# tuanggolt/hyperdrive

Hardware: AMD Instinct MI355X
Metric: verified consensus msgs/sec (secp256k1) at 1/2/4/8 MI355X; % INT32 VALU peak (higher is better)
Workload: dtype u32 (256-bit modular integer arithmetic)

## Files before the change

hyperdrive_amd/_lib.py:

```python
from __future__ import annotations

import atexit
import ctypes
import os
import weakref

HERE = os.path.dirname(os.path.abspath(__file__))
LIB_PATH = os.environ.get("HD_LIB", os.path.join(HERE, "_lib", "libhdverify.so"))

HD_OK = 0
HD_EINVAL = -1
HD_ENOMEM = -2
HD_EDEVICE = -3
HD_ECAP = -4
HD_EAGAIN = -5

c_u8p = ctypes.POINTER(ctypes.c_uint8)
c_i8p = ctypes.POINTER(ctypes.c_int8)
c_i64p = ctypes.POINTER(ctypes.c_int64)
c_u32p = ctypes.POINTER(ctypes.c_uint32)
c_i32p = ctypes.POINTER(ctypes.c_int32)


class HdBatch(ctypes.Structure):
# ... 87 lines not shown
                ("done", ctypes.c_void_p)]


SIGNATURES = {
    "hd_ctx_create": (ctypes.c_int, [ctypes.c_int, ctypes.POINTER(ctypes.c_void_p)]),
    "hd_ctx_destroy": (ctypes.c_int, [ctypes.c_void_p]),
    "hd_ctx_set_pubkey_format": (ctypes.c_int, [ctypes.c_void_p, ctypes.c_int]),
    "hd_set_signatories": (ctypes.c_int, [ctypes.c_void_p, ctypes.c_void_p, ctypes.c_uint32]),
    "hd_ctx_set_fastpath": (ctypes.c_int, [ctypes.c_void_p, ctypes.c_int]),
    "hd_ctx_fastpath_stats": (ctypes.c_int, [ctypes.c_void_p, ctypes.POINTER(ctypes.c_uint32),
                                             ctypes.POINTER(ctypes.c_uint32)]),
    "hd_ctx_foreign_stats": (ctypes.c_int, [ctypes.c_void_p, ctypes.POINTER(ctypes.c_uint32),
                                            ctypes.POINTER(ctypes.c_uint32), ctypes.POINTER(ctypes.c_uint32)]),
    "hd_ctx_dedup_stats": (ctypes.c_int, [ctypes.c_void_p, ctypes.POINTER(ctypes.c_uint64),
                                          ctypes.POINTER(ctypes.c_uint64)]),
    "hd_ctx_fastpath_geometry": (ctypes.c_int, [ctypes.c_void_p, ctypes.POINTER(ctypes.c_int),
                                                ctypes.POINTER(ctypes.c_int), ctypes.POINTER(ctypes.c_int)]),
    "hd_ctx_profile": (ctypes.c_int, [ctypes.c_void_p, ctypes.c_int]),
    "hd_ctx_set_variant": (ctypes.c_int, [ctypes.c_void_p, ctypes.c_int, ctypes.c_int]),
    "hd_ctx_get_variant": (ctypes.c_int, [ctypes.c_void_p, ctypes.c_int, ctypes.POINTER(ctypes.c_int)]),
    "hd_ctx_profile_read": (ctypes.c_int, [ctypes.c_void_p, ctypes.POINTER(ctypes.c_uint32),
                                           ctypes.POINTER(ctypes.c_double), ctypes.POINTER(ctypes.c_uint32),
                                           ctypes.POINTER(ctypes.c_double)]),
    "hd_verify_batch": (ctypes.c_int, [ctypes.c_void_p, ctypes.POINTER(HdBatch), ctypes.c_void_p,
                                       ctypes.c_void_p, ctypes.c_void_p]),
    "hd_verify_batch_device": (ctypes.c_int, [ctypes.c_void_p, ctypes.POINTER(HdBatch), ctypes.c_void_p,
                                              ctypes.c_void_p, ctypes.c_void_p, ctypes.c_void_p, ctypes.c_void_p]),
    "hd_authenticate_batch_device": (ctypes.c_int, [ctypes.c_void_p, ctypes.POINTER(HdBatch), ctypes.c_void_p,
                                                    ctypes.c_void_p]),
    "hd_verify_submit": (ctypes.c_int, [ctypes.c_void_p, ctypes.POINTER(HdBatch), ctypes.c_void_p, ctypes.c_void_p,
# ... 174 lines not shown
```

hyperdrive_amd/csrc/hd_dedup.h:

```cpp
#pragma once
#include "hd_common.h"

namespace hd {

#define HD_DD_PROBES 8u
#define HD_DD_EMPTY 0xFFFFFFFFu
#define HD_DD_REPEAT 0x80000000u
#define HD_DD_FINAL 0xC0000000u
#define HD_DD_INDEX 0x3FFFFFFFu
#define HD_DD_MAX_N (1u << 30)

struct DdKey {
    int64_t height, round;
    uint32_t value[8], from[8], r[8], s[8];
    uint32_t v;
};

HD bool dd_key_equal(const DdKey& a, const DdKey& b) {
    uint32_t d = (uint32_t)(a.height != b.height) | (uint32_t)(a.round != b.round) | (a.v ^ b.v);
    HD_UNROLL for (int k = 0; k < 8; k++)
        d |= (a.value[k] ^ b.value[k]) | (a.from[k] ^ b.from[k]) | (a.r[k] ^ b.r[k]) | (a.s[k] ^ b.s[k]);
    return d == 0;
}

HD void dd_key_load(DdKey& k, const int64_t* height, const int64_t* round, const uint8_t* value32,
                    const uint8_t* digest32, const uint8_t* from32, const uint8_t* sig65, size_t i, size_t n) {
    if (digest32) {
        k.height = k.round = 0;
        load_row32_be(k.value, digest32, i);
    } else {
        k.height = height[i];
        k.round = round[i];
        load_row32_be(k.value, value32, i);
    }
    load_row32_be(k.from, from32, i);
    load_sig65(k.r, k.s, k.v, sig65, i, n);
}

HD uint32_t dd_hash(const DdKey& k) {
    uint32_t h = k.r[0] * 0x9E3779B1u;
    h = (h ^ k.r[7]) * 0x85EBCA6Bu;
    h = (h ^ (h >> 15) ^ k.s[0]) * 0xC2B2AE35u;
    h = (h ^ k.s[7]) * 0x27D4EB2Fu;
    h = (h ^ (h >> 13) ^ k.from[0]) * 0x165667B1u;
    h = (h ^ k.from[7]) * 0x9E3779B1u;
    return h ^ (h >> 16);
}

HD uint32_t dd_table_words(uint32_t n) {
    uint32_t w = 1024u;
    while (w < 4u * (uint64_t)n && w < 0x80000000u) w <<= 1;
    return w;
}

}
```

hyperdrive_amd/csrc/hd_fastverify.hip:

```cpp
#include <hip/hip_runtime.h>

#include <algorithm>
#include <cstdio>
#include <cstdlib>
#include <cstring>
#include <string>
#include <map>
#include <mutex>
#include <unordered_map>
#include <vector>

#include "../../include/hd_verify.h"
#include "hd_fixedbase.h"
#include "hd_dedup.h"
#include "hd_scmont.h"
#include "hd_internal.h"
#include "hd_verify_msg.h"

using namespace hd;

struct FbWork {
    const gp* gtab = nullptr;
    uint32_t nslots = 0;
    uint32_t max_slots = 0;
// ... 1 lines not shown
    std::vector<gp*> chunks;
    ge* base = nullptr;
    ge* pub = nullptr;
    uint32_t* state = nullptr;
    int32_t* adm_slot = nullptr;
    bool map_ok = true;
    size_t cap_adm_slot = 0;
    uint32_t* list = nullptr;
    uint32_t* counts = nullptr;
    uint32_t* zr = nullptr;
    struct Scratch {
        uint32_t* rows = nullptr;
        size_t cap_rows = 0;
        uint32_t* dtab = nullptr;
        size_t cap_dtab = 0;
        uint32_t* slow = nullptr;
        size_t cap_slow = 0;
        uint32_t* count = nullptr;
        uint32_t* slow2 = nullptr;
        size_t cap_slow2 = 0;
        hipEvent_t done = nullptr;
        hipStream_t stream = nullptr;
        bool used = false;
    };
    static constexpr int NSCRATCH = 3;
    Scratch sc[NSCRATCH];
    int next = 0;
    int last_set = -1;
    uint32_t* nr_host = nullptr;
    uint32_t* nr_dev = nullptr;
    uint32_t* est_host = nullptr;
    uint32_t* est_dev = nullptr;
    unsigned long long* dstats = nullptr;
    hipEvent_t done = nullptr;
    hipStream_t last = nullptr;
    bool any = false;
    bool steady = false;
    bool prof = false;
    std::vector<hipEvent_t> ev_call, ev_sums;
    size_t n_call = 0, n_sums = 0;
    std::unordered_map<std::string, uint32_t> slot_of;
    std::vector<uint32_t> free_slots;
    uint32_t used = 1;
    int wp = HD_FB_W;
    int last_k = 8;
    double budget = 0;
    size_t bytes = 0;
    uint32_t* fdict = nullptr;
// ... 74 lines not shown
    if (p == 1) __builtin_amdgcn_s_setprio(1);
    else if (p == 2) __builtin_amdgcn_s_setprio(2);
    else if (p >= 3) __builtin_amdgcn_s_setprio(3);
}

#define HD_REF_NEG 0x80000000u
#define HD_REF_ZERO 0x40000000u
#define HD_REF_IDX 0x3FFFFFFFu
template <int W>
HD uint32_t fb_ref(int d, int w) {
    const uint32_t ad = (uint32_t)(d < 0 ? -d : d);
    const uint32_t base = (uint32_t)w * FbL<W>::N;
    return d == 0 ? (base | HD_REF_ZERO) : ((base + ad - 1) | (d < 0 ? HD_REF_NEG : 0u));
}

__global__ __launch_bounds__(256) void k_fast_prep(DevBatch b, const uint8_t* __restrict__ digest_in,
                                                   const uint32_t* __restrict__ state,
                                                   const int32_t* __restrict__ adm_slot, AdmIndex ix,
                                                   uint32_t n_adm, SplitRows rows, const uint32_t* __restrict__ fdict,
                                                   uint32_t* __restrict__ fhit, uint32_t fbase,
                                                   uint32_t* __restrict__ dtab, uint32_t dmask) {
    wave_prio(rows.prio);
    const uint32_t i = blockIdx.x * blockDim.x + threadIdx.x;
    const uint32_t n = b.n;
    const bool present = i < n;
    FastSrc src{b, present ? i : 0u, digest_in};
    const uint32_t type = present ? src.type() : 0u;
    uint32_t code = HD_NEEDS_SLOW, slot = 0, rep = HD_DD_EMPTY;
    int32_t idx = -1;
    sc r, s, m;
    if (!present) {
    } else if (type < 1 || type > 3) {
        code = V_BAD_TYPE;
    } else {
        uint32_t from_be[8];
        src.from_words(from_be);
        idx = n_adm ? adm_index_find(ix, from_be) : -1;
        int32_t sl = idx >= 0 ? adm_slot[idx] : -1;
        if (idx < 0 && fdict) {
            sl = fdict_find(fdict, from_be);
            if (sl >= 0) idx = -2;
        }
        if (sl >= 0 && state[sl] == HD_FB_READY) {
            slot = (uint32_t)sl;
            if (idx == -2) atomicAdd(&fhit[sl - (int32_t)fbase], 1u);
            FastIn in;
            DdKey me;
            me.height = me.round = 0;
            if (digest_in) {
                load_row32_be(in.digest_be, digest_in, i);
                HD_UNROLL for (int k = 0; k < 8; k++) me.value[k] = in.digest_be[k];
            } else {
                src.value_words(me.value);
                me.height = b.height[i];
                me.round = b.round[i];
                if (type == T_PROPOSE)
                    sha256_propose(in.digest_be, me.height, me.round, b.valid_round ? b.valid_round[i] : -1, me.value);
                else
                    sha256_vote(in.digest_be, me.height, me.round, me.value);
            }
            src.sig(in.r_be, in.s_be, in.v);
            in.ready = true;
            fe x;
            uint8_t o;
            if (fast_prefix(o, r, s, m, x, in)) {
                code = HD_FAST_LIVE;
                if (dtab && type != T_PROPOSE) {
                    HD_UNROLL for (int k = 0; k < 8; k++) {
                        me.from[k] = from_be[k];
                        me.r[k] = in.r_be[k];
                        me.s[k] = in.s_be[k];
                    }
                    me.v = in.v;
                    const uint32_t h = dd_hash(me);
                    HD_NOUNROLL for (uint32_t p = 0; p < HD_DD_PROBES; p++) {
                        const uint32_t cur = atomicCAS(&dtab[(h + p) & dmask], HD_DD_EMPTY, i);
                        if (cur == HD_DD_EMPTY) break;
                        DdKey other;
                        dd_key_load(other, b.height, b.round, b.value32, digest_in, b.from32, b.sig65, cur, n);
                        if (dd_key_equal(me, other)) {
                            rep = cur;
                            break;
                        }
                    }
                }
            } else {
                code = o;
            }
        }
    }
    const bool live = code == HD_FAST_LIVE;
    const bool distinct = live && rep == HD_DD_EMPTY;
    __shared__ uint32_t s_cnt[4], s_base;
    const uint32_t lane = threadIdx.x & 63u, wv = threadIdx.x >> 6;
    const unsigned long long bd = __ballot(distinct), br = __ballot(live && !distinct);
// ... 798 lines not shown
    if (const char* m = getenv("HD_FB_MAX_BYTES")) f->budget = atof(m);
    f->max_slots = (uint32_t)std::max(1.0, std::min(1e6, f->budget / fb_slot_bytes(f->wp)));
    FBCHK(hipMalloc(&f->counts, 8), "fb counts");
    FBCHK(hipMalloc(&f->zr, fb_run_scratch_bytes(ctx)), "fb builder scratch");
    FBCHK(hipHostMalloc((void**)&f->nr_host, 4, hipHostMallocMapped | hipHostMallocCoherent), "fb ready count");
    *f->nr_host = 0xFFFFFFFFu;
    FBCHK(hipHostGetDevicePointer((void**)&f->nr_dev, f->nr_host, 0), "fb ready count map");
    FBCHK(hipHostMalloc((void**)&f->est_host, 16, hipHostMallocMapped | hipHostMallocCoherent), "fb list estimate");
    f->est_host[0] = f->est_host[1] = f->est_host[2] = f->est_host[3] = 0xFFFFFFFFu;
    FBCHK(hipHostGetDevicePointer((void**)&f->est_dev, f->est_host, 0), "fb list estimate map");
    FBCHK(hipHostMalloc((void**)&f->fpend_host, 8, hipHostMallocMapped | hipHostMallocCoherent), "fb foreign claims");
    f->fpend_host[0] = f->fpend_host[1] = 0;
    FBCHK(hipHostGetDevicePointer((void**)&f->fpend_dev, f->fpend_host, 0), "fb foreign claims map");
    FBCHK(hipMalloc(&f->dstats, 16), "fb repeat counters");
    FBCHK(hipMemset(f->dstats, 0, 16), "fb repeat counters clear");
    int rc = fb_alloc_slots(ctx);
    if (rc) return rc;
    return fb_g_table(ctx, &f->gtab);
}

const gp* hd_fb_gtab(const hd_ctx* ctx) { return ctx && ctx->fb ? ctx->fb->gtab : nullptr; }

void hd_fb_release(hd_ctx* ctx) {
    if (!ctx || !ctx->fb) return;
    FbWork* f = ctx->fb;
    fb_free_tables(ctx);
    if (f->done) (void)hipEventDestroy(f->done);
    for (hipEvent_t e : f->ev_call) (void)hipEventDestroy(e);
    for (hipEvent_t e : f->ev_sums) (void)hipEventDestroy(e);
    for (auto& sc : f->sc) {
        if (sc.done) (void)hipEventDestroy(sc.done);
        void* sp[] = {sc.rows, sc.slow, sc.count, sc.slow2, sc.dtab};
        for (void* p : sp)
            if (p) (void)hipFree(p);
    }
    void* ptrs[] = {f->counts, f->adm_slot, f->zr, f->fdict, f->fnext, f->fhit, f->fkey, f->dstats};
    for (void* p : ptrs)
        if (p) (void)hipFree(p);
    if (f->nr_host) (void)hipHostFree(f->nr_host);
    if (f->est_host) (void)hipHostFree(f->est_host);
    if (f->fpend_host) (void)hipHostFree(f->fpend_host);
    delete f;
    ctx->fb = nullptr;
}

static int split_k_for(const hd_ctx* ctx, uint32_t n) {
    const int k = ctx->var[HD_VAR_SPLIT_K];
    if (k > 0) return k;
    uint64_t lanes = n;
    if (const volatile uint32_t* est = ctx->fb->est_host) {
        const uint32_t seen = est[2], of = est[3];
// ... 190 lines not shown
    const int pf = ctx->var[HD_VAR_SUM_PREFETCH];
    if (w == 0) w = (uint64_t)n < 2ull * 3 * 4 * 64 * (uint64_t)std::max(ctx->n_cu, 1) ? 4 : 3;
    if (pf == 2) {
        if (w == 2) k_fast_sums<2, WP, 2><<<blocks, 256, 0, s>>>(n, gtab, tab, rows);
        else k_fast_sums<3, WP, 2><<<blocks, 256, 0, s>>>(n, gtab, tab, rows);
    } else {
        if (w == 2) k_fast_sums<2, WP, 1><<<blocks, 256, 0, s>>>(n, gtab, tab, rows);
        else if (w == 4) k_fast_sums<4, WP, 0><<<blocks, 256, 0, s>>>(n, gtab, tab, rows);
        else k_fast_sums<3, WP, 1><<<blocks, 256, 0, s>>>(n, gtab, tab, rows);
    }
}

template <int K, int WP>
static void launch_split(hd_ctx* ctx, const DevBatch& b, const uint8_t* d_digest, uint8_t* d_verdict,
                         uint8_t* d_rec32, int32_t* d_signer, uint32_t* d_bitmap, const SplitRows& rows,
                         const FbWork::Scratch& sc, hipStream_t s, bool auth) {
    FbWork* f = ctx->fb;
    const uint32_t n = b.n;
    const uint32_t tb = (split_lanes<K>(n) + 255) / 256, nb = (n + 255) / 256;
    uint32_t* dtab = ctx->var[HD_VAR_DEDUP] ? sc.dtab : nullptr;
    k_fast_prep<<<nb, 256, 0, s>>>(b, d_digest, f->state, f->adm_slot, hd_adm_index(ctx), ctx->n_adm, rows,
                                   f->fcap ? f->fdict : nullptr, f->fhit, f->fbase, dtab, dd_table_words(n) - 1u);
    k_fast_sinv<K><<<tb, 256, 0, s>>>(n, rows, f->est_dev + 2, f->dstats);
    hipEvent_t* pe = fb_prof_pair(f->ev_sums, f->n_sums, f->prof);
    if (pe) (void)hipEventRecord(pe[0], s);
    launch_sums<WP>(ctx, nb, s, n, f->gtab, f->tabs, rows);
    if (pe) (void)hipEventRecord(pe[1], s);
    k_fast_zinv<K><<<tb, 256, 0, s>>>(n, rows);
    k_fast_cmp<<<nb, 256, 0, s>>>(b, rows, ctx->d_adm_perm, d_verdict, d_rec32, d_signer, sc.slow, sc.count,
                                  d_bitmap, auth);
}

static int fb_verify_impl(hd_ctx* ctx, const DevBatch& b, const uint8_t* d_digest, uint8_t* d_verdict,
                          uint8_t* d_rec32, int32_t* d_signer, uint32_t* d_bitmap, FbWork::Scratch& sc,
                          hipStream_t s, bool auth);

int hd_fb_verify(hd_ctx* ctx, const DevBatch& b, const uint8_t* d_digest, uint8_t* d_verdict, uint8_t* d_rec32,
                 int32_t* d_signer, uint32_t* d_bitmap, hipStream_t s, bool auth) {
    FbWork* f = ctx->fb;
    if (!f->done) FBCHK(hipEventCreateWithFlags(&f->done, hipEventDisableTiming), "fb event");
    const int j = f->next;
    f->next = (j + 1) % FbWork::NSCRATCH;
    FbWork::Scratch& sc = f->sc[j];
    if (!sc.done) FBCHK(hipEventCreateWithFlags(&sc.done, hipEventDisableTiming), "fb scratch event");
    if (!sc.count) FBCHK(hipMalloc(&sc.count, 16), "fb scratch count");
    bool evicted = false;
    int re = fb_evict(ctx, &evicted);
    if (re) return re;
    const bool steady = !evicted && f->nr_host && *(volatile uint32_t*)f->nr_host == 0 && !fb_foreign_pending(f);
    if (sc.used && sc.stream != s) FBCHK(hipStreamWaitEvent(s, sc.done, 0), "fb scratch order");
    if (f->any && f->last != s && !(steady && f->steady)) FBCHK(hipStreamWaitEvent(s, f->done, 0), "fb stream order");
    hipEvent_t* pe = fb_prof_pair(f->ev_call, f->n_call, f->prof);
    if (pe) (void)hipEventRecord(pe[0], s);
    const int rc = fb_verify_impl(ctx, b, d_digest, d_verdict, d_rec32, d_signer, d_bitmap, sc, s, auth);
    if (pe) (void)hipEventRecord(pe[1], s);
    FBCHK(hipEventRecord(sc.done, s), "fb scratch record");
    FBCHK(hipEventRecord(f->done, s), "fb event record");
    sc.used = true;
    sc.stream = s;
    f->last_set = j;
// ... 9 lines not shown
    for (auto& sc : f->sc)
        if (sc.used) FBCHK(hipEventSynchronize(sc.done), "fb quiesce");
    if (f->any) FBCHK(hipEventSynchronize(f->done), "fb quiesce");
    return HD_OK;
}

static int fb_verify_impl(hd_ctx* ctx, const DevBatch& b, const uint8_t* d_digest, uint8_t* d_verdict,
                          uint8_t* d_rec32, int32_t* d_signer, uint32_t* d_bitmap, FbWork::Scratch& sc,
                          hipStream_t s, bool auth) {
    FbWork* f = ctx->fb;
    int rc = hd_dev_grow(ctx, (void**)&sc.slow, &sc.cap_slow, 4 * (size_t)b.n);
    if (rc) return rc;
    const uint32_t blocks = (b.n + 255) / 256;
    rc = hd_dev_grow(ctx, (void**)&sc.slow2, &sc.cap_slow2, 4 * (size_t)b.n);
    if (rc) return rc;
    FBCHK(hipMemsetAsync(sc.count, 0, 16, s), "fb count reset");
    if (ctx->n_adm > 0 && f->adm_slot && f->map_ok) {
        if (b.n > HD_DD_MAX_N) {
            ctx->last_error = "known-key check: more than 2^30 messages in one call";
            return HD_EINVAL;
        }
        const size_t row_words = 63;
        rc = hd_dev_grow(ctx, (void**)&sc.rows, &sc.cap_rows, 4 * row_words * (size_t)b.n);
        if (rc) return rc;
        const uint32_t n = b.n;
        if (ctx->var[HD_VAR_DEDUP]) {
            const size_t tab_bytes = 4 * (size_t)dd_table_words(n);
            rc = hd_dev_grow(ctx, (void**)&sc.dtab, &sc.cap_dtab, tab_bytes);
            if (rc) return rc;
            FBCHK(hipMemsetAsync(sc.dtab, 0xFF, tab_bytes, s), "fb repeat table clear");
        }
        SplitRows rows;
        rows.aux = sc.rows;
        rows.idx = (int32_t*)(sc.rows + (size_t)n);
        rows.u1 = sc.rows + 2 * (size_t)n;
        rows.u2 = sc.rows + 10 * (size_t)n;
        rows.s = sc.rows + 18 * (size_t)n;
        rows.pre = sc.rows + 26 * (size_t)n;
        rows.xyz = sc.rows + 35 * (size_t)n;
        rows.ref = sc.rows + 62 * (size_t)n;
        rows.cnt = sc.count;
        rows.prio = ctx->var[HD_VAR_WAVE_PRIO];
        const int k = split_k_for(ctx, n);
        f->last_k = k;
#define HD_SPLIT(K, WP) launch_split<K, WP>(ctx, b, d_digest, d_verdict, d_rec32, d_signer, d_bitmap, rows, sc, s, auth)
        if (f->wp == HD_FB_WX) {
            if (k == 16) HD_SPLIT(16, HD_FB_WX);
            else HD_SPLIT(8, HD_FB_WX);
        } else if (f->wp == HD_FB_WW) {
            if (k == 16) HD_SPLIT(16, HD_FB_WW);
            else HD_SPLIT(8, HD_FB_WW);
        } else if (f->wp == HD_FB_WN) {
            if (k == 16) HD_SPLIT(16, HD_FB_WN);
            else HD_SPLIT(8, HD_FB_WN);
        } else {
            if (k == 16) HD_SPLIT(16, HD_FB_W);
            else HD_SPLIT(8, HD_FB_W);
        }
#undef HD_SPLIT
        FBCHK(hipGetLastError(), "split check launch");
// ... 129 lines not shown
int hd_ctx_dedup_stats(hd_ctx* ctx, uint64_t* checked, uint64_t* repeats) {
    if (!ctx) return HD_EINVAL;
    if (checked) *checked = 0;
    if (repeats) *repeats = 0;
    if (!ctx->fb || !ctx->fb->dstats) return HD_OK;
    (void)hipSetDevice(ctx->device);
    int rq = hd_ctx_quiesce(ctx);
    if (rq) return rq;
    unsigned long long st[2] = {0, 0};
    FBCHK(hipMemcpy(st, ctx->fb->dstats, 16, hipMemcpyDeviceToHost), "repeat counters read");
    if (checked) *checked = st[0];
    if (repeats) *repeats = st[1];
    return HD_OK;
}

}
```

hyperdrive_amd/csrc/hd_internal.h:

```cpp
#pragma once
#include <hip/hip_runtime.h>

#include <string>
#include <utility>
#include <vector>

#include "../../include/hd_verify.h"
#include "hd_fixedbase.h"
#include "hd_verify_msg.h"

struct DevBatch {
    uint32_t n;
    const uint8_t* type;
    const int64_t* height;
    const int64_t* round;
    const int64_t* valid_round;
    const uint8_t* value32;
    const uint8_t* from32;
    const uint8_t* sig65;
};

enum BufSlot {
    BUF_TYPE, BUF_HEIGHT, BUF_ROUND, BUF_VROUND, BUF_VALUE, BUF_FROM, BUF_SIG,
    BUF_VERDICT, BUF_REC, BUF_SIGNER, BUF_BITMAP, BUF_DUP, BUF__COUNT
};

struct DevBuf {
    void* p = nullptr;
    size_t cap = 0;
};

struct TallyWork;
struct HostPipe;
struct FbWork;

struct hd_ctx {
    int device = 0;
    int n_cu = 256;
    int verify_waves = 3;
    int var[HD_VAR__COUNT] = {3, 0, 1, 0, -1, 0, 2, 0, 0, 0, 16, 1, 1, 0, 0};
    hipStream_t stream = nullptr;
    int pkfmt = HD_PUBKEY_COMPRESSED;
    hd::ge* d_gtab = nullptr;
    uint32_t* d_adm = nullptr;
    int32_t* d_adm_perm = nullptr;
    size_t cap_adm = 0, cap_adm_perm = 0;
    uint32_t n_adm = 0;
    uint32_t adm_ver = 0;
    uint8_t* d_sig_caller = nullptr;
    size_t cap_sig_caller = 0;
    uint32_t n_sig_caller = 0;
    int adm_steps = 0;
    uint32_t* d_adm_ix = nullptr;
    size_t cap_adm_ix = 0;
    uint32_t adm_ix_mask = 0;
// ... 67 lines not shown
```

hyperdrive_amd/csrc/hd_verify.hip:

```cpp
#include <hip/hip_runtime.h>

#include <algorithm>
#include <cstdio>
#include <cstdlib>
#include <cstring>
#include <mutex>
#include <string>
#include <vector>

#include "../../include/hd_digest.h"
#include "../../include/hd_verify.h"
#include "hd_fixedbase.h"
#include "hd_verify_msg.h"
#include "hd_internal.h"

using namespace hd;

struct DevSrc {
    const DevBatch& b;
    uint32_t i;
    const uint8_t* dg;
    __device__ __forceinline__ uint32_t type() const { return b.type[i]; }
    __device__ __forceinline__ int64_t h() const { return b.height[i]; }
    __device__ __forceinline__ int64_t r() const { return b.round[i]; }
// ... 174 lines not shown
    ctx->device = device;
    hipError_t e = hipSetDevice(device);
    if (e == hipSuccess) e = hipStreamCreateWithFlags(&ctx->stream, hipStreamNonBlocking);
    if (e != hipSuccess) {
        int rc = hd_ctx_fail(ctx, e, "hipStreamCreate");
        delete ctx;
        return rc;
    }
    hipDeviceProp_t prop;
    if (hipGetDeviceProperties(&prop, device) == hipSuccess) ctx->n_cu = prop.multiProcessorCount;
    struct { int key; const char* env; } envs[] = {
        {HD_VAR_VERIFY_WAVES, "HD_VERIFY_WAVES"}, {HD_VAR_SUM_WAVES, "HD_SUM_WAVES"},
        {HD_VAR_SUM_PREFETCH, "HD_SUM_PF"},       {HD_VAR_SPLIT_K, "HD_FAST_K"},
        {HD_VAR_KEY_WIDTH, "HD_FB_PW"},           {HD_VAR_WAVE_PRIO, "HD_WAVE_PRIO"},
        {HD_VAR_FOREIGN_KEYS, "HD_FOREIGN_KEYS"}, {HD_VAR_SLOW_LIFT, "HD_SLOW_LIFT"},
        {HD_VAR_DEDUP, "HD_DEDUP"},
    };
    for (auto& ev : envs)
        if (const char* e = getenv(ev.env)) (void)hd_ctx_set_variant(ctx, ev.key, atoi(e));
    if (getenv("HD_RECOVER_GLV_G")) (void)hd_ctx_set_variant(ctx, HD_VAR_RECOVER_G, 1);
    if (const char* f = getenv("HD_VERIFY_FASTPATH")) ctx->fastpath = atoi(f) != 0;
    static std::once_flag once;
    static std::vector<ge> host_tab(2 * HD_GLV_GTAB_N);
    std::call_once(once, [] { build_gtab_glv(host_tab.data()); });
    e = hipMalloc(&ctx->d_gtab, sizeof(ge) * 2 * HD_GLV_GTAB_N);
    if (e == hipSuccess)
        e = hipMemcpy(ctx->d_gtab, host_tab.data(), sizeof(ge) * 2 * HD_GLV_GTAB_N, hipMemcpyHostToDevice);
    if (e != hipSuccess) {
        int rc = hd_ctx_fail(ctx, e, "gtab upload");
        hd_ctx_destroy(ctx);
        return rc;
// ... 27 lines not shown
    hd_host_release(ctx);
    hd_tally_release(ctx);
    hd_fb_release(ctx);
    if (ctx->stream) (void)hipStreamDestroy(ctx->stream);
    delete ctx;
    return HD_OK;
}

int hd_ctx_set_variant(hd_ctx* ctx, int which, int value) {
    if (!ctx || which < 0 || which >= HD_VAR__COUNT) return HD_EINVAL;
    bool ok = false;
    switch (which) {
        case HD_VAR_VERIFY_WAVES: ok = value >= 2 && value <= 4; break;
        case HD_VAR_SUM_WAVES: ok = value == 0 || (value >= 2 && value <= 4); break;
        case HD_VAR_SUM_PREFETCH: ok = value == 1 || value == 2; break;
        case HD_VAR_RECOVER_G: case HD_VAR_SLOW_LIFT: case HD_VAR_DEDUP: ok = value == 0 || value == 1; break;
        case HD_VAR_SPLIT_K: ok = value == -1 || value == 8 || value == 16; break;
        case HD_VAR_KEY_WIDTH:
            ok = value == 0 || value == HD_FB_W || value == HD_FB_WW || value == HD_FB_WN || value == HD_FB_WX;
            break;
        case HD_VAR_WAVE_PRIO: ok = value >= 0 && value <= 3; break;
        case HD_VAR_FOREIGN_KEYS: ok = value >= 0 && value <= 64; break;
        default: ok = false;
    }
    if (!ok) return HD_EINVAL;
    ctx->var[which] = value;
    if (which == HD_VAR_VERIFY_WAVES) ctx->verify_waves = value;
    return HD_OK;
}

int hd_ctx_get_variant(hd_ctx* ctx, int which, int* value) {
// ... 224 lines not shown
```

hyperdrive_amd/verify.py:

```python
from __future__ import annotations

import ctypes
from dataclasses import dataclass
from typing import Dict, List, Optional, Sequence, Tuple

import numpy as np

from . import _lib
from ._lib import HDError, HdBatch, HdTallyOut

VALID = 0
BAD_RECID = 1
BAD_RS = 2
NO_POINT = 3
INFINITY = 4
SIGNATORY_MISMATCH = 5
NOT_ADMITTED = 6
BAD_TYPE = 7
NOT_AUTHENTIC = 8
VERDICT_NAMES = ["VALID", "BAD_RECID", "BAD_RS", "NO_POINT", "INFINITY", "SIGNATORY_MISMATCH",
                 "NOT_ADMITTED", "BAD_TYPE", "NOT_AUTHENTIC"]

PROPOSE, PREVOTE, PRECOMMIT = 1, 2, 3

# ... 326 lines not shown
        return self

    def __exit__(self, *exc):
        self.close()

    @property
    def handle(self):
        return self._ctx

    def set_signatories(self, signatories) -> None:
        arr = _as_rows(signatories, 32)
        self._check(self._lib.hd_set_signatories(self._ctx, _ptr(arr), len(arr)), "hd_set_signatories")
        self.n_signatories = len(arr)

    VARIANTS = {"verify_waves": 0, "sum_waves": 1, "sum_prefetch": 2, "split_k": 4, "recover_g": 5,
                "key_width": 7, "wave_prio": 8, "foreign_keys": 10, "slow_lift": 11, "dedup": 12}

    def set_variant(self, name: str, value: int) -> None:
        self._check(self._lib.hd_ctx_set_variant(self._ctx, self.VARIANTS[name], int(value)), "hd_ctx_set_variant")

    def variant(self, name: str) -> int:
        v = ctypes.c_int()
        self._check(self._lib.hd_ctx_get_variant(self._ctx, self.VARIANTS[name], ctypes.byref(v)), "hd_ctx_get_variant")
        return v.value

    def set_fastpath(self, enable: bool) -> None:
        self._check(self._lib.hd_ctx_set_fastpath(self._ctx, 1 if enable else 0), "hd_ctx_set_fastpath")

    def profile(self, enable: bool) -> None:
        self._check(self._lib.hd_ctx_profile(self._ctx, 1 if enable else 0), "hd_ctx_profile")

# ... 8 lines not shown
        k, f = ctypes.c_uint32(), ctypes.c_uint32()
        self._check(self._lib.hd_ctx_fastpath_stats(self._ctx, ctypes.byref(k), ctypes.byref(f)),
                    "hd_ctx_fastpath_stats")
        return int(k.value), int(f.value)

    def foreign_stats(self, checks: bool = False):
        r, e, c = ctypes.c_uint32(), ctypes.c_uint32(), ctypes.c_uint32()
        self._check(self._lib.hd_ctx_foreign_stats(self._ctx, ctypes.byref(r), ctypes.byref(e), ctypes.byref(c)),
                    "hd_ctx_foreign_stats")
        return (int(r.value), int(e.value), int(c.value)) if checks else (int(r.value), int(e.value))

    def dedup_stats(self) -> Tuple[int, int]:
        c, r = ctypes.c_uint64(), ctypes.c_uint64()
        self._check(self._lib.hd_ctx_dedup_stats(self._ctx, ctypes.byref(c), ctypes.byref(r)), "hd_ctx_dedup_stats")
        return int(c.value), int(r.value)

    def fastpath_geometry(self) -> Tuple[int, int, int]:
        g, k, m = ctypes.c_int(), ctypes.c_int(), ctypes.c_int()
        self._check(self._lib.hd_ctx_fastpath_geometry(self._ctx, ctypes.byref(g), ctypes.byref(k), ctypes.byref(m)),
                    "hd_ctx_fastpath_geometry")
        return int(g.value), int(k.value), int(m.value)

    def known_keys(self) -> int:
        return self.fastpath_stats()[0]

    def verify_batch(self, batch: Batch, recovered: bool = True) -> VerifyResult:
        n = len(batch)
        verdict = np.zeros(n, np.uint8)
        rec = np.zeros((n, 32), np.uint8)
        bitmap = np.zeros((n + 31) // 32, np.uint32)
# ... 259 lines not shown
```

include/hd_verify.h:

```cpp
#ifndef HD_VERIFY_H
#define HD_VERIFY_H

#include <stddef.h>
#include <stdint.h>

#ifdef __cplusplus
extern "C" {
#endif

#define HD_OK 0
#define HD_EINVAL (-1)
#define HD_ENOMEM (-2)
#define HD_EDEVICE (-3)
#define HD_ECAP (-4)
#define HD_EAGAIN (-5)

#define HD_TYPE_PROPOSE 1
#define HD_TYPE_PREVOTE 2
#define HD_TYPE_PRECOMMIT 3

#define HD_VERDICT_VALID 0
#define HD_VERDICT_BAD_RECID 1
#define HD_VERDICT_BAD_RS 2
#define HD_VERDICT_NO_POINT 3
// ... 16 lines not shown
    const uint8_t* sig65;
} hd_batch;

int hd_ctx_create(int device, hd_ctx** out);
int hd_ctx_destroy(hd_ctx* ctx);
#define HD_PUBKEY_UNCOMPRESSED 0
#define HD_PUBKEY_COMPRESSED 1
#define HD_PUBKEY_RAW64 2
#define HD_PUBKEY_XY_STRIPPED 3
int hd_ctx_set_pubkey_format(hd_ctx* ctx, int format);
int hd_set_signatories(hd_ctx* ctx, const uint8_t* sigs32, uint32_t n);
int hd_ctx_set_fastpath(hd_ctx* ctx, int enable);
int hd_ctx_fastpath_stats(hd_ctx* ctx, uint32_t* known_keys, uint32_t* last_fallback);
int hd_ctx_foreign_stats(hd_ctx* ctx, uint32_t* ready_slots, uint32_t* evictions, uint32_t* checks);
int hd_ctx_dedup_stats(hd_ctx* ctx, uint64_t* checked, uint64_t* repeats);
int hd_ctx_fastpath_geometry(hd_ctx* ctx, int* g_windows, int* key_windows, int* msgs_per_inversion);
int hd_ctx_profile(hd_ctx* ctx, int enable);
#define HD_VAR_VERIFY_WAVES 0
#define HD_VAR_SUM_WAVES 1
#define HD_VAR_SUM_PREFETCH 2
#define HD_VAR_SPLIT_K 4
#define HD_VAR_RECOVER_G 5
#define HD_VAR_KEY_WIDTH 7
#define HD_VAR_WAVE_PRIO 8
#define HD_VAR_FOREIGN_KEYS 10
#define HD_VAR_SLOW_LIFT 11
#define HD_VAR_DEDUP 12
#define HD_VAR__COUNT 15
int hd_ctx_set_variant(hd_ctx* ctx, int which, int value);
int hd_ctx_get_variant(hd_ctx* ctx, int which, int* value);
int hd_ctx_profile_read(hd_ctx* ctx, uint32_t* calls, double* verify_ms, uint32_t* sums_launches, double* sums_ms);

int hd_verify_batch(hd_ctx* ctx, const hd_batch* batch, uint8_t* verdict, uint8_t* recovered32,
                    uint32_t* valid_bitmap);

int hd_verify_batch_device(hd_ctx* ctx, const hd_batch* dbatch, uint8_t* d_verdict, uint8_t* d_recovered32,
                           int32_t* d_signer, uint32_t* d_valid_bitmap, void* stream);

int hd_authenticate_batch_device(hd_ctx* ctx, const hd_batch* dbatch, uint8_t* d_verdict, void* stream);

#define HD_HOST_SLOTS 3
int hd_verify_submit(hd_ctx* ctx, const hd_batch* batch, uint8_t* verdict, uint8_t* recovered32,
                     uint32_t* valid_bitmap, uint64_t* ticket);
// ... 162 lines not shown
```

Baseline: 1.056 billion.

## Share SHA-256 preimage digests across messages with identical vote content

Adds a pre-pass that hashes each message's (type, height, round, valid_round, value) tuple into a table. Within each wave it uses shuffles to collapse runs of identical neighbours, so only one SHA-256 digest is computed per distinct preimage. The fast-prep kernel then loads the shared digest by id, and the repeat-signature check compares preimage ids instead of reloading full keys. This removes redundant hashing when many validators vote on the same value, but adds two extra kernel launches, a second table clear and atomics, all enabled by default.

```diff
diff --git a/hyperdrive_amd/_lib.py b/hyperdrive_amd/_lib.py
--- a/hyperdrive_amd/_lib.py
+++ b/hyperdrive_amd/_lib.py
@@ -125,6 +125,8 @@
                                             ctypes.POINTER(ctypes.c_uint32), ctypes.POINTER(ctypes.c_uint32)]),
     "hd_ctx_dedup_stats": (ctypes.c_int, [ctypes.c_void_p, ctypes.POINTER(ctypes.c_uint64),
                                           ctypes.POINTER(ctypes.c_uint64)]),
+    "hd_ctx_preimage_stats": (ctypes.c_int, [ctypes.c_void_p, ctypes.POINTER(ctypes.c_uint64),
+                                             ctypes.POINTER(ctypes.c_uint64)]),
     "hd_ctx_fastpath_geometry": (ctypes.c_int, [ctypes.c_void_p, ctypes.POINTER(ctypes.c_int),
                                                 ctypes.POINTER(ctypes.c_int), ctypes.POINTER(ctypes.c_int)]),
     "hd_ctx_profile": (ctypes.c_int, [ctypes.c_void_p, ctypes.c_int]),
diff --git a/hyperdrive_amd/csrc/hd_dedup.h b/hyperdrive_amd/csrc/hd_dedup.h
--- a/hyperdrive_amd/csrc/hd_dedup.h
+++ b/hyperdrive_amd/csrc/hd_dedup.h
@@ -37,15 +37,16 @@
     load_sig65(k.r, k.s, k.v, sig65, i, n);
 }
 
-HD uint32_t dd_hash(const DdKey& k) {
-    uint32_t h = k.r[0] * 0x9E3779B1u;
-    h = (h ^ k.r[7]) * 0x85EBCA6Bu;
-    h = (h ^ (h >> 15) ^ k.s[0]) * 0xC2B2AE35u;
-    h = (h ^ k.s[7]) * 0x27D4EB2Fu;
-    h = (h ^ (h >> 13) ^ k.from[0]) * 0x165667B1u;
-    h = (h ^ k.from[7]) * 0x9E3779B1u;
+HD uint32_t dd_hash_words(uint32_t r0, uint32_t r7, uint32_t s0, uint32_t s7, uint32_t f0, uint32_t f7) {
+    uint32_t h = r0 * 0x9E3779B1u;
+    h = (h ^ r7) * 0x85EBCA6Bu;
+    h = (h ^ (h >> 15) ^ s0) * 0xC2B2AE35u;
+    h = (h ^ s7) * 0x27D4EB2Fu;
+    h = (h ^ (h >> 13) ^ f0) * 0x165667B1u;
+    h = (h ^ f7) * 0x9E3779B1u;
     return h ^ (h >> 16);
 }
+HD uint32_t dd_hash(const DdKey& k) { return dd_hash_words(k.r[0], k.r[7], k.s[0], k.s[7], k.from[0], k.from[7]); }
 
 HD uint32_t dd_table_words(uint32_t n) {
     uint32_t w = 1024u;
@@ -53,4 +54,48 @@
     return w;
 }
 
+struct DdPre {
+    uint32_t is_propose;
+    int64_t valid_round;
+    int64_t height, round;
+    uint32_t value[8];
+};
+
+HD void dd_pre_load(DdPre& k, bool is_propose, const int64_t* height, const int64_t* round, const int64_t* vround,
+                    const uint8_t* value32, size_t i) {
+    k.is_propose = is_propose ? 1u : 0u;
+    k.valid_round = is_propose ? (vround ? vround[i] : -1) : 0;
+    k.height = height[i];
+    k.round = round[i];
+    load_row32_be(k.value, value32, i);
 }
+
+HD bool dd_pre_equal(const DdPre& a, const DdPre& b) {
+    uint32_t d = (a.is_propose ^ b.is_propose) | (uint32_t)(a.valid_round != b.valid_round) |
+                 (uint32_t)(a.height != b.height) | (uint32_t)(a.round != b.round);
+    HD_UNROLL for (int k = 0; k < 8; k++) d |= a.value[k] ^ b.value[k];
+    return d == 0;
+}
+
+HD uint32_t dd_pre_hash(const DdPre& k) {
+    uint32_t h = ((uint32_t)(uint64_t)k.height) * 0x9E3779B1u;
+    h = (h ^ (uint32_t)((uint64_t)k.height >> 32)) * 0x85EBCA6Bu;
+    h = (h ^ (h >> 15) ^ (uint32_t)(uint64_t)k.round) * 0xC2B2AE35u;
+    h = (h ^ (uint32_t)((uint64_t)k.round >> 32)) * 0x27D4EB2Fu;
+    h = (h ^ (h >> 13) ^ k.value[0]) * 0x165667B1u;
+    h = (h ^ k.value[7]) * 0x9E3779B1u;
+    h = (h ^ (h >> 14) ^ k.is_propose ^ ((uint32_t)(uint64_t)k.valid_round << 1)) * 0x85EBCA6Bu;
+    return h ^ (h >> 16);
+}
+
+HD bool dd_pid_is_ref(uint32_t q) { return (q >> 30) == 2u; }
+HD bool dd_pid_is_none(uint32_t q) { return (q >> 30) == 3u; }
+HD uint32_t dd_pid_claimant(uint32_t q) { return q & HD_DD_INDEX; }
+HD uint32_t dd_pid_ref(uint32_t claimant) { return HD_DD_REPEAT | claimant; }
+HD uint32_t dd_pid_resolve(const uint32_t* pid, uint32_t i) {
+    uint32_t q = pid[i];
+    if (dd_pid_is_ref(q)) q = pid[dd_pid_claimant(q)];
+    return q;
+}
+
+}
diff --git a/hyperdrive_amd/csrc/hd_fastverify.hip b/hyperdrive_amd/csrc/hd_fastverify.hip
--- a/hyperdrive_amd/csrc/hd_fastverify.hip
+++ b/hyperdrive_amd/csrc/hd_fastverify.hip
@@ -39,6 +39,8 @@
         size_t cap_rows = 0;
         uint32_t* dtab = nullptr;
         size_t cap_dtab = 0;
+        uint8_t* pre = nullptr;
+        size_t cap_pre = 0;
         uint32_t* slow = nullptr;
         size_t cap_slow = 0;
         uint32_t* count = nullptr;
@@ -57,6 +59,7 @@
     uint32_t* est_host = nullptr;
     uint32_t* est_dev = nullptr;
     unsigned long long* dstats = nullptr;
+    unsigned long long* pstats = nullptr;
     hipEvent_t done = nullptr;
     hipStream_t last = nullptr;
     bool any = false;
@@ -161,12 +164,114 @@
     return d == 0 ? (base | HD_REF_ZERO) : ((base + ad - 1) | (d < 0 ? HD_REF_NEG : 0u));
 }
 
+struct PreRows {
+    uint8_t* dig;
+    uint32_t* pid;
+    uint32_t* plist;
+    uint32_t* cnt;
+};
+
+#define HD_PRE_BLOCK 1024
+__global__ __launch_bounds__(HD_PRE_BLOCK) void k_pre_claim(DevBatch b, PreRows pre, uint32_t* __restrict__ ptab,
+                                                   uint32_t pmask, int prio) {
+    wave_prio(prio);
+    const uint32_t i = blockIdx.x * blockDim.x + threadIdx.x;
+    const bool present = i < b.n;
+    const uint32_t type = present ? b.type[i] : 0u;
+    const bool typed = type >= 1 && type <= 3;
+    const uint32_t lane = threadIdx.x & 63u, wv = threadIdx.x >> 6;
+    uint32_t rep = HD_DD_EMPTY, h = 0;
+    DdPre me;
+    me.is_propose = 0;
+    me.valid_round = me.height = me.round = 0;
+    HD_UNROLL for (int k = 0; k < 8; k++) me.value[k] = 0;
+    if (typed) {
+        dd_pre_load(me, type == T_PROPOSE, b.height, b.round, b.valid_round, b.value32, i);
+        h = dd_pre_hash(me);
+    }
+    auto probe = [&]() -> bool {
+        HD_NOUNROLL for (uint32_t p = 0; p < HD_DD_PROBES; p++) {
+            const uint32_t cur = atomicCAS(&ptab[(h + p) & pmask], HD_DD_EMPTY, i);
+            if (cur == HD_DD_EMPTY) return true;
+            DdPre other;
+            dd_pre_load(other, b.type[cur] == T_PROPOSE, b.height, b.round, b.valid_round, b.value32, cur);
+            if (dd_pre_equal(me, other)) {
+                rep = cur;
+                return true;
+            }
+        }
+        return false;
+    };
+    auto up = [&](uint32_t x) { return (uint32_t)__shfl_up((int)x, 1); };
+    auto up64 = [&](int64_t x) {
+        return (int64_t)((uint64_t)up((uint32_t)((uint64_t)x >> 32)) << 32 | up((uint32_t)(uint64_t)x));
+    };
+    DdPre pk;
+    pk.is_propose = up(me.is_propose);
+    pk.valid_round = up64(me.valid_round);
+    pk.height = up64(me.height);
+    pk.round = up64(me.round);
+    HD_UNROLL for (int k = 0; k < 8; k++) pk.value[k] = up(me.value[k]);
+    const bool prev_typed = up(typed ? 1u : 0u) != 0u;
+    const bool head = typed && (lane == 0 || !prev_typed || !dd_pre_equal(me, pk));
+    uint32_t found = 0;
+    if (head) found = probe() ? 1u : 0u;
+    const unsigned long long hm = __ballot(head) & ((2ull << lane) - 1ull);
+    const int hl = hm ? 63 - __clzll((long long)hm) : 0;
+    const uint32_t hrep = (uint32_t)__shfl((int)rep, hl), hfound = (uint32_t)__shfl((int)found, hl);
+    if (typed && !head && hfound) rep = hrep == HD_DD_EMPTY ? i - lane + (uint32_t)hl : hrep;
+    const bool claimant = typed && rep == HD_DD_EMPTY;
+    __shared__ uint32_t s_cnt[HD_PRE_BLOCK / 64], s_base;
+    const unsigned long long bc = __ballot(claimant), bu = __ballot(present && !typed);
+    if (lane == 0) s_cnt[wv] = (uint32_t)__popcll(bc) | (uint32_t)__popcll(bu) << 16;
+    __syncthreads();
+    if (threadIdx.x == 0) {
+        uint32_t t = 0;
+        for (uint32_t w = 0; w < HD_PRE_BLOCK / 64; w++) t += s_cnt[w];
+        s_base = 0;
+        if (t & 0xFFFFu) s_base = atomicAdd(pre.cnt + 4, t & 0xFFFFu);
+        if (t >> 16) atomicAdd(pre.cnt + 5, t >> 16);
+    }
+    __syncthreads();
+    if (!present) return;
+    if (claimant) {
+        uint32_t id = s_base + (uint32_t)__popcll(bc & ((1ull << lane) - 1ull));
+        for (uint32_t w = 0; w < wv; w++) id += s_cnt[w] & 0xFFFFu;
+        pre.plist[id] = i;
+        pre.pid[i] = id;
+    } else {
+        pre.pid[i] = typed ? dd_pid_ref(rep) : HD_DD_FINAL;
+    }
+}
+
+__global__ __launch_bounds__(256) void k_pre_hash(DevBatch b, PreRows pre, unsigned long long* __restrict__ stats,
+                                                  int prio) {
+    wave_prio(prio);
+    const uint32_t id = blockIdx.x * blockDim.x + threadIdx.x;
+    const uint32_t nd = pre.cnt[4];
+    if (id == 0) {
+        const uint32_t typed = b.n - pre.cnt[5];
+        if (typed) atomicAdd(&stats[0], (unsigned long long)typed);
+        if (nd) atomicAdd(&stats[1], (unsigned long long)nd);
+    }
+    if (id >= nd) return;
+    const uint32_t i = pre.plist[id];
+    uint32_t value[8], out[8];
+    load_row32_be(value, b.value32, i);
+    if (b.type[i] == T_PROPOSE)
+        sha256_propose(out, b.height[i], b.round[i], b.valid_round ? b.valid_round[i] : -1, value);
+    else
+        sha256_vote(out, b.height[i], b.round[i], value);
+    store_row32_be(pre.dig, id, out);
+}
+
+template <bool SHARE>
 __global__ __launch_bounds__(256) void k_fast_prep(DevBatch b, const uint8_t* __restrict__ digest_in,
                                                    const uint32_t* __restrict__ state,
                                                    const int32_t* __restrict__ adm_slot, AdmIndex ix,
                                                    uint32_t n_adm, SplitRows rows, const uint32_t* __restrict__ fdict,
                                                    uint32_t* __restrict__ fhit, uint32_t fbase,
-                                                   uint32_t* __restrict__ dtab, uint32_t dmask) {
+                                                   uint32_t* __restrict__ dtab, uint32_t dmask, PreRows pre) {
     wave_prio(rows.prio);
     const uint32_t i = blockIdx.x * blockDim.x + threadIdx.x;
     const uint32_t n = b.n;
@@ -193,8 +298,12 @@
             if (idx == -2) atomicAdd(&fhit[sl - (int32_t)fbase], 1u);
             FastIn in;
             DdKey me;
+            uint32_t my_id = 0;
             me.height = me.round = 0;
-            if (digest_in) {
+            if constexpr (SHARE) {
+                my_id = dd_pid_resolve(pre.pid, i);
+                load_row32_be(in.digest_be, pre.dig, my_id);
+            } else if (digest_in) {
                 load_row32_be(in.digest_be, digest_in, i);
                 HD_UNROLL for (int k = 0; k < 8; k++) me.value[k] = in.digest_be[k];
             } else {
@@ -213,19 +322,32 @@
             if (fast_prefix(o, r, s, m, x, in)) {
                 code = HD_FAST_LIVE;
                 if (dtab && type != T_PROPOSE) {
-                    HD_UNROLL for (int k = 0; k < 8; k++) {
-                        me.from[k] = from_be[k];
-                        me.r[k] = in.r_be[k];
-                        me.s[k] = in.s_be[k];
+                    if constexpr (!SHARE) {
+                        HD_UNROLL for (int k = 0; k < 8; k++) {
+                            me.from[k] = from_be[k];
+                            me.r[k] = in.r_be[k];
+                            me.s[k] = in.s_be[k];
+                        }
+                        me.v = in.v;
                     }
-                    me.v = in.v;
-                    const uint32_t h = dd_hash(me);
+                    const uint32_t h = dd_hash_words(in.r_be[0], in.r_be[7], in.s_be[0], in.s_be[7], from_be[0], from_be[7]);
                     HD_NOUNROLL for (uint32_t p = 0; p < HD_DD_PROBES; p++) {
                         const uint32_t cur = atomicCAS(&dtab[(h + p) & dmask], HD_DD_EMPTY, i);
                         if (cur == HD_DD_EMPTY) break;
-                        DdKey other;
-                        dd_key_load(other, b.height, b.round, b.value32, digest_in, b.from32, b.sig65, cur, n);
-                        if (dd_key_equal(me, other)) {
+                        bool eq;
+                        if constexpr (SHARE) {
+                            uint32_t d = dd_pid_resolve(pre.pid, cur) ^ my_id, w[8], w2[8], v2;
+                            load_row32_be(w, b.from32, cur);
+                            HD_UNROLL for (int k = 0; k < 8; k++) d |= w[k] ^ from_be[k];
+                            load_sig65(w, w2, v2, b.sig65, cur, n);
+                            HD_UNROLL for (int k = 0; k < 8; k++) d |= (w[k] ^ in.r_be[k]) | (w2[k] ^ in.s_be[k]);
+                            eq = (d | (v2 ^ in.v)) == 0;
+                        } else {
+                            DdKey other;
+                            dd_key_load(other, b.height, b.round, b.value32, digest_in, b.from32, b.sig65, cur, n);
+                            eq = dd_key_equal(me, other);
+                        }
+                        if (eq) {
                             rep = cur;
                             break;
                         }
@@ -1054,6 +1176,8 @@
     FBCHK(hipHostGetDevicePointer((void**)&f->fpend_dev, f->fpend_host, 0), "fb foreign claims map");
     FBCHK(hipMalloc(&f->dstats, 16), "fb repeat counters");
     FBCHK(hipMemset(f->dstats, 0, 16), "fb repeat counters clear");
+    FBCHK(hipMalloc(&f->pstats, 16), "fb preimage counters");
+    FBCHK(hipMemset(f->pstats, 0, 16), "fb preimage counters clear");
     int rc = fb_alloc_slots(ctx);
     if (rc) return rc;
     return fb_g_table(ctx, &f->gtab);
@@ -1070,11 +1194,11 @@
     for (hipEvent_t e : f->ev_sums) (void)hipEventDestroy(e);
     for (auto& sc : f->sc) {
         if (sc.done) (void)hipEventDestroy(sc.done);
-        void* sp[] = {sc.rows, sc.slow, sc.count, sc.slow2, sc.dtab};
+        void* sp[] = {sc.rows, sc.slow, sc.count, sc.slow2, sc.dtab, sc.pre};
         for (void* p : sp)
             if (p) (void)hipFree(p);
     }
-    void* ptrs[] = {f->counts, f->adm_slot, f->zr, f->fdict, f->fnext, f->fhit, f->fkey, f->dstats};
+    void* ptrs[] = {f->counts, f->adm_slot, f->zr, f->fdict, f->fnext, f->fhit, f->fkey, f->dstats, f->pstats};
     for (void* p : ptrs)
         if (p) (void)hipFree(p);
     if (f->nr_host) (void)hipHostFree(f->nr_host);
@@ -1295,13 +1419,23 @@
 template <int K, int WP>
 static void launch_split(hd_ctx* ctx, const DevBatch& b, const uint8_t* d_digest, uint8_t* d_verdict,
                          uint8_t* d_rec32, int32_t* d_signer, uint32_t* d_bitmap, const SplitRows& rows,
-                         const FbWork::Scratch& sc, hipStream_t s, bool auth) {
+                         const FbWork::Scratch& sc, hipStream_t s, bool auth, bool share) {
     FbWork* f = ctx->fb;
     const uint32_t n = b.n;
     const uint32_t tb = (split_lanes<K>(n) + 255) / 256, nb = (n + 255) / 256;
+    const uint32_t tw = dd_table_words(n);
     uint32_t* dtab = ctx->var[HD_VAR_DEDUP] ? sc.dtab : nullptr;
-    k_fast_prep<<<nb, 256, 0, s>>>(b, d_digest, f->state, f->adm_slot, hd_adm_index(ctx), ctx->n_adm, rows,
-                                   f->fcap ? f->fdict : nullptr, f->fhit, f->fbase, dtab, dd_table_words(n) - 1u);
+    const uint32_t* fdict = f->fcap ? f->fdict : nullptr;
+    if (share) {
+        const PreRows pre{sc.pre, (uint32_t*)(sc.pre + 32 * (size_t)n), (uint32_t*)(sc.pre + 36 * (size_t)n), sc.count};
+        k_pre_claim<<<(n + HD_PRE_BLOCK - 1) / HD_PRE_BLOCK, HD_PRE_BLOCK, 0, s>>>(b, pre, sc.dtab + tw, tw - 1u, rows.prio);
+        k_pre_hash<<<nb, 256, 0, s>>>(b, pre, f->pstats, rows.prio);
+        k_fast_prep<true><<<nb, 256, 0, s>>>(b, nullptr, f->state, f->adm_slot, hd_adm_index(ctx), ctx->n_adm, rows,
+                                             fdict, f->fhit, f->fbase, dtab, tw - 1u, pre);
+    } else {
+        k_fast_prep<false><<<nb, 256, 0, s>>>(b, d_digest, f->state, f->adm_slot, hd_adm_index(ctx), ctx->n_adm, rows,
+                                              fdict, f->fhit, f->fbase, dtab, tw - 1u, PreRows{});
+    }
     k_fast_sinv<K><<<tb, 256, 0, s>>>(n, rows, f->est_dev + 2, f->dstats);
     hipEvent_t* pe = fb_prof_pair(f->ev_sums, f->n_sums, f->prof);
     if (pe) (void)hipEventRecord(pe[0], s);
@@ -1324,7 +1458,7 @@
     f->next = (j + 1) % FbWork::NSCRATCH;
     FbWork::Scratch& sc = f->sc[j];
     if (!sc.done) FBCHK(hipEventCreateWithFlags(&sc.done, hipEventDisableTiming), "fb scratch event");
-    if (!sc.count) FBCHK(hipMalloc(&sc.count, 16), "fb scratch count");
+    if (!sc.count) FBCHK(hipMalloc(&sc.count, 32), "fb scratch count");
     bool evicted = false;
     int re = fb_evict(ctx, &evicted);
     if (re) return re;
@@ -1364,7 +1498,7 @@
     const uint32_t blocks = (b.n + 255) / 256;
     rc = hd_dev_grow(ctx, (void**)&sc.slow2, &sc.cap_slow2, 4 * (size_t)b.n);
     if (rc) return rc;
-    FBCHK(hipMemsetAsync(sc.count, 0, 16, s), "fb count reset");
+    FBCHK(hipMemsetAsync(sc.count, 0, 32, s), "fb count reset");
     if (ctx->n_adm > 0 && f->adm_slot && f->map_ok) {
         if (b.n > HD_DD_MAX_N) {
             ctx->last_error = "known-key check: more than 2^30 messages in one call";
@@ -1374,11 +1508,17 @@
         rc = hd_dev_grow(ctx, (void**)&sc.rows, &sc.cap_rows, 4 * row_words * (size_t)b.n);
         if (rc) return rc;
         const uint32_t n = b.n;
-        if (ctx->var[HD_VAR_DEDUP]) {
+        const bool share = ctx->var[HD_VAR_PRE_SHARE] && !d_digest;
+        if (ctx->var[HD_VAR_DEDUP] || share) {
             const size_t tab_bytes = 4 * (size_t)dd_table_words(n);
-            rc = hd_dev_grow(ctx, (void**)&sc.dtab, &sc.cap_dtab, tab_bytes);
+            rc = hd_dev_grow(ctx, (void**)&sc.dtab, &sc.cap_dtab, 2 * tab_bytes);
             if (rc) return rc;
-            FBCHK(hipMemsetAsync(sc.dtab, 0xFF, tab_bytes, s), "fb repeat table clear");
+            const size_t first = ctx->var[HD_VAR_DEDUP] ? 0 : tab_bytes, last = share ? 2 * tab_bytes : tab_bytes;
+            FBCHK(hipMemsetAsync((uint8_t*)sc.dtab + first, 0xFF, last - first, s), "fb table clear");
+        }
+        if (share) {
+            rc = hd_dev_grow(ctx, (void**)&sc.pre, &sc.cap_pre, 40 * (size_t)n);
+            if (rc) return rc;
         }
         SplitRows rows;
         rows.aux = sc.rows;
@@ -1393,7 +1533,7 @@
         rows.prio = ctx->var[HD_VAR_WAVE_PRIO];
         const int k = split_k_for(ctx, n);
         f->last_k = k;
-#define HD_SPLIT(K, WP) launch_split<K, WP>(ctx, b, d_digest, d_verdict, d_rec32, d_signer, d_bitmap, rows, sc, s, auth)
+#define HD_SPLIT(K, WP) launch_split<K, WP>(ctx, b, d_digest, d_verdict, d_rec32, d_signer, d_bitmap, rows, sc, s, auth, share)
         if (f->wp == HD_FB_WX) {
             if (k == 16) HD_SPLIT(16, HD_FB_WX);
             else HD_SPLIT(8, HD_FB_WX);
@@ -1553,4 +1693,19 @@
     return HD_OK;
 }
 
-}
+int hd_ctx_preimage_stats(hd_ctx* ctx, uint64_t* typed, uint64_t* distinct) {
+    if (!ctx) return HD_EINVAL;
+    if (typed) *typed = 0;
+    if (distinct) *distinct = 0;
+    if (!ctx->fb || !ctx->fb->pstats) return HD_OK;
+    (void)hipSetDevice(ctx->device);
+    int rq = hd_ctx_quiesce(ctx);
+    if (rq) return rq;
+    unsigned long long st[2] = {0, 0};
+    FBCHK(hipMemcpy(st, ctx->fb->pstats, 16, hipMemcpyDeviceToHost), "preimage counters read");
+    if (typed) *typed = st[0];
+    if (distinct) *distinct = st[1];
+    return HD_OK;
+}
+
+}
diff --git a/hyperdrive_amd/csrc/hd_internal.h b/hyperdrive_amd/csrc/hd_internal.h
--- a/hyperdrive_amd/csrc/hd_internal.h
+++ b/hyperdrive_amd/csrc/hd_internal.h
@@ -38,7 +38,7 @@
     int device = 0;
     int n_cu = 256;
     int verify_waves = 3;
-    int var[HD_VAR__COUNT] = {3, 0, 1, 0, -1, 0, 2, 0, 0, 0, 16, 1, 1, 0, 0};
+    int var[HD_VAR__COUNT] = {3, 0, 1, 0, -1, 0, 2, 0, 0, 0, 16, 1, 1, 0, 0, 1};
     hipStream_t stream = nullptr;
     int pkfmt = HD_PUBKEY_COMPRESSED;
     hd::ge* d_gtab = nullptr;
diff --git a/hyperdrive_amd/csrc/hd_verify.hip b/hyperdrive_amd/csrc/hd_verify.hip
--- a/hyperdrive_amd/csrc/hd_verify.hip
+++ b/hyperdrive_amd/csrc/hd_verify.hip
@@ -212,7 +212,7 @@
         {HD_VAR_SUM_PREFETCH, "HD_SUM_PF"},       {HD_VAR_SPLIT_K, "HD_FAST_K"},
         {HD_VAR_KEY_WIDTH, "HD_FB_PW"},           {HD_VAR_WAVE_PRIO, "HD_WAVE_PRIO"},
         {HD_VAR_FOREIGN_KEYS, "HD_FOREIGN_KEYS"}, {HD_VAR_SLOW_LIFT, "HD_SLOW_LIFT"},
-        {HD_VAR_DEDUP, "HD_DEDUP"},
+        {HD_VAR_DEDUP, "HD_DEDUP"},               {HD_VAR_PRE_SHARE, "HD_PRE_SHARE"},
     };
     for (auto& ev : envs)
         if (const char* e = getenv(ev.env)) (void)hd_ctx_set_variant(ctx, ev.key, atoi(e));
@@ -270,7 +270,9 @@
         case HD_VAR_VERIFY_WAVES: ok = value >= 2 && value <= 4; break;
         case HD_VAR_SUM_WAVES: ok = value == 0 || (value >= 2 && value <= 4); break;
         case HD_VAR_SUM_PREFETCH: ok = value == 1 || value == 2; break;
-        case HD_VAR_RECOVER_G: case HD_VAR_SLOW_LIFT: case HD_VAR_DEDUP: ok = value == 0 || value == 1; break;
+        case HD_VAR_RECOVER_G: case HD_VAR_SLOW_LIFT: case HD_VAR_DEDUP: case HD_VAR_PRE_SHARE:
+            ok = value == 0 || value == 1;
+            break;
         case HD_VAR_SPLIT_K: ok = value == -1 || value == 8 || value == 16; break;
         case HD_VAR_KEY_WIDTH:
             ok = value == 0 || value == HD_FB_W || value == HD_FB_WW || value == HD_FB_WN || value == HD_FB_WX;
diff --git a/hyperdrive_amd/verify.py b/hyperdrive_amd/verify.py
--- a/hyperdrive_amd/verify.py
+++ b/hyperdrive_amd/verify.py
@@ -364,7 +364,8 @@
         self.n_signatories = len(arr)
 
     VARIANTS = {"verify_waves": 0, "sum_waves": 1, "sum_prefetch": 2, "split_k": 4, "recover_g": 5,
-                "key_width": 7, "wave_prio": 8, "foreign_keys": 10, "slow_lift": 11, "dedup": 12}
+                "key_width": 7, "wave_prio": 8, "foreign_keys": 10, "slow_lift": 11, "dedup": 12,
+                "pre_share": 15}
 
     def set_variant(self, name: str, value: int) -> None:
         self._check(self._lib.hd_ctx_set_variant(self._ctx, self.VARIANTS[name], int(value)), "hd_ctx_set_variant")
@@ -403,6 +404,12 @@
         c, r = ctypes.c_uint64(), ctypes.c_uint64()
         self._check(self._lib.hd_ctx_dedup_stats(self._ctx, ctypes.byref(c), ctypes.byref(r)), "hd_ctx_dedup_stats")
         return int(c.value), int(r.value)
+
+    def preimage_stats(self) -> Tuple[int, int]:
+        t, d = ctypes.c_uint64(), ctypes.c_uint64()
+        self._check(self._lib.hd_ctx_preimage_stats(self._ctx, ctypes.byref(t), ctypes.byref(d)),
+                    "hd_ctx_preimage_stats")
+        return int(t.value), int(d.value)
 
     def fastpath_geometry(self) -> Tuple[int, int, int]:
         g, k, m = ctypes.c_int(), ctypes.c_int(), ctypes.c_int()
diff --git a/include/hd_verify.h b/include/hd_verify.h
--- a/include/hd_verify.h
+++ b/include/hd_verify.h
@@ -54,6 +54,7 @@
 int hd_ctx_fastpath_stats(hd_ctx* ctx, uint32_t* known_keys, uint32_t* last_fallback);
 int hd_ctx_foreign_stats(hd_ctx* ctx, uint32_t* ready_slots, uint32_t* evictions, uint32_t* checks);
 int hd_ctx_dedup_stats(hd_ctx* ctx, uint64_t* checked, uint64_t* repeats);
+int hd_ctx_preimage_stats(hd_ctx* ctx, uint64_t* typed, uint64_t* distinct);
 int hd_ctx_fastpath_geometry(hd_ctx* ctx, int* g_windows, int* key_windows, int* msgs_per_inversion);
 int hd_ctx_profile(hd_ctx* ctx, int enable);
 #define HD_VAR_VERIFY_WAVES 0
@@ -66,7 +67,8 @@
 #define HD_VAR_FOREIGN_KEYS 10
 #define HD_VAR_SLOW_LIFT 11
 #define HD_VAR_DEDUP 12
-#define HD_VAR__COUNT 15
+#define HD_VAR_PRE_SHARE 15
+#define HD_VAR__COUNT 16
 int hd_ctx_set_variant(hd_ctx* ctx, int which, int value);
 int hd_ctx_get_variant(hd_ctx* ctx, int which, int* value);
 int hd_ctx_profile_read(hd_ctx* ctx, uint32_t* calls, double* verify_ms, uint32_t* sums_launches, double* sums_ms);
```

Result: faster. 1.069 billion, median of 6 (+1.2%).
